# GATB/gatb-core

Hardware: AMD Instinct MI355X
Metric: distinct k-mers/s at k=31 (higher is better)
Workload: dtype u64

## Files before the change

gatb-core_amd/csrc/gkc_common.hpp:

```cpp
#pragma once
#include <hip/hip_runtime.h>
#include <stdint.h>
#include <stdio.h>
#include <stdlib.h>
#include <stdarg.h>
#include <string.h>
#include <string>
#include <vector>
#include <chrono>
#include <map>
#include <atomic>
#include <mutex>
#include <condition_variable>
#include <thread>
#include <algorithm>
#include "../../include/gkc.h"

struct gkc_error { int code; std::string msg; };

#define GKC_FAIL(ctx, code_, ...) do { (ctx)->set_error((code_), __VA_ARGS__); return (code_); } while (0)
#define GKC_HIP(ctx, call) do { hipError_t e_ = (call); if (e_ != hipSuccess) { \
    (ctx)->set_error(e_ == hipErrorOutOfMemory ? GKC_ERR_NOMEM : GKC_ERR_HIP, "%s failed: %s (%s:%d)", #call, hipGetErrorString(e_), __FILE__, __LINE__); \
    return e_ == hipErrorOutOfMemory ? GKC_ERR_NOMEM : GKC_ERR_HIP; } } while (0)
#define GKC_TRY(expr) do { int rc_ = (expr); if (rc_ != GKC_OK) return rc_; } while (0)

constexpr uint64_t GKC_PASS_GATHERED = 0x6761746865726564ull;
constexpr int SCAN_THREADS = 512;
constexpr int SCAN_PER_THREAD = 16;
constexpr int SCAN_TILE = SCAN_THREADS * SCAN_PER_THREAD;
constexpr int DESC_START_BITS = 13, DESC_NBK_BITS = 6;
static_assert(SCAN_TILE == (1 << DESC_START_BITS), "descriptor start field");
constexpr uint32_t DESC_PARTS_MAX = 1u << (32 - DESC_START_BITS - DESC_NBK_BITS);
constexpr uint32_t SCAN_COARSE_MAX = 4096;
constexpr int SCAN_HALO_WORDS = 4;
constexpr int SCAN_WORDS = SCAN_TILE / 16 + SCAN_HALO_WORDS;

constexpr int MAX_SUB_BITS = 13;
constexpr int MAX_SUB = 1 << MAX_SUB_BITS;
constexpr int SUB_TARGET = 512;

struct GkcTun {
    uint32_t scan_coarse_max; uint64_t push_split, push_chunk; bool scan_global_atomics, refine_recompute, scan_no_desc;
    int weight_bits, dedupe, max_sub_bits, lanes; uint64_t slice_min, batch_keys; bool slices, batch_lpt, no_f64; uint32_t wg_max, scatter_wgs, deep_bits, sink_first_div;
    bool sink_packed, sink_packed2, sink_width6, sink_two_widths, sink_debug; int sink_adaptive; uint64_t sink_dense; int unpack_threads;
    bool bloom_atomic, bloom_gather, mphf_regions, mphf_ordered; uint64_t bloom_query_regions_min, mphf_regions_min;
    uint64_t query_index_stride;
    int vmm; uint32_t vmm_chunk_mb, vmm_min_mb; bool vmm_with_rccl, pool_debug, pool_trace, verbose; double filebox_timeout; char fault[32];
    static const char* raw(const char* name) { return getenv(name); }
    static long long num(const char* name, long long dflt) { const char* e = raw(name); return e && *e ? atoll(e) : dflt; }
    static bool on(const char* name) { return raw(name) != nullptr; }
    static bool not0(const char* name) { const char* e = raw(name); return !(e && atoi(e) == 0); }
    void read() {
        scan_coarse_max = (uint32_t)std::max<long long>(1, num("GKC_SCAN_COARSE_MAX", SCAN_COARSE_MAX));
        push_split = (uint64_t)std::max<long long>(1024, num("GKC_PUSH_SPLIT", 16000000000ll)); push_chunk = (uint64_t)std::max<long long>(64, num("GKC_PUSH_CHUNK", 1ll << 30));
        scan_global_atomics = on("GKC_SCAN_GLOBAL_ATOMICS"); refine_recompute = on("GKC_REFINE_RECOMPUTE"); scan_no_desc = on("GKC_SCAN_NO_DESC");
        weight_bits = (int)num("GKC_WEIGHT_BITS", 0); dedupe = (int)num("GKC_DEDUPE", -1); max_sub_bits = (int)num("GKC_MAX_SUB_BITS", -1); lanes = (int)num("GKC_STAGEB_LANES", 2);
        slice_min = (uint64_t)std::max<long long>(1, num("GKC_SLICE_MIN", 8000000)); batch_keys = (uint64_t)num("GKC_BATCH_KEYS", 0);
        slices = not0("GKC_SLICES"); batch_lpt = not0("GKC_BATCH_LPT"); no_f64 = on("GKC_NO_F64");
        wg_max = (uint32_t)num("GKC_WG_MAX", 0); scatter_wgs = (uint32_t)std::max<long long>(1, num("GKC_SCATTER_WGS", 176)); deep_bits = (uint32_t)std::max<long long>(1, num("GKC_DEEP_BITS", MAX_SUB_BITS));
        sink_first_div = (uint32_t)std::max<long long>(1, num("GKC_SINK_FIRST_DIV", 4));
        sink_packed = not0("GKC_SINK_PACKED"); sink_packed2 = not0("GKC_SINK_PACKED2"); sink_width6 = not0("GKC_SINK_WIDTH6"); sink_debug = on("GKC_SINK_DEBUG"); sink_adaptive = (int)num("GKC_SINK_ADAPTIVE", 1);
        sink_two_widths = not0("GKC_SINK_TWO_WIDTHS");
        sink_dense = (uint64_t)num("GKC_SINK_DENSE", 0); unpack_threads = (int)num("GKC_UNPACK_THREADS", 0);
        bloom_atomic = on("GKC_BLOOM_ATOMIC"); bloom_gather = on("GKC_BLOOM_GATHER"); mphf_regions = not0("GKC_MPHF_REGIONS"); mphf_ordered = on("GKC_MPHF_ORDERED");
        bloom_query_regions_min = (uint64_t)num("GKC_BLOOM_QUERY_REGIONS_MIN", 2000000); mphf_regions_min = (uint64_t)num("GKC_MPHF_REGIONS_MIN", 1ll << 21);
        query_index_stride = (uint64_t)std::min<long long>(1ll << 40, std::max<long long>(1, num("GKC_QUERY_INDEX_STRIDE", 256)));
        vmm = (int)num("GKC_VMM", 1); vmm_chunk_mb = (uint32_t)std::max<long long>(2, num("GKC_VMM_CHUNK_MB", 1024)); vmm_min_mb = (uint32_t)std::max<long long>(1, num("GKC_VMM_MIN_MB", 64));
        vmm_with_rccl = num("GKC_VMM_WITH_RCCL", 0) == 1; pool_debug = on("GKC_POOL_DEBUG"); pool_trace = on("GKC_POOL_TRACE"); verbose = on("GKC_VERBOSE");
        filebox_timeout = raw("GKC_FILEBOX_TIMEOUT") ? atof(raw("GKC_FILEBOX_TIMEOUT")) : 600.0; memset(fault, 0, sizeof fault); if (raw("GKC_FAULT")) strncpy(fault, raw("GKC_FAULT"), sizeof fault - 1);
    }
};
inline GkcTun& gkc_tun() { static GkcTun t = [] { GkcTun x; x.read(); return x; }(); return t; }
inline void gkc_tun_refresh() { static std::mutex mu; std::lock_guard<std::mutex> lk(mu); GkcTun x; x.read(); gkc_tun() = x; }

inline thread_local hipStream_t tl_stream_ = nullptr;

struct VmmBlock { size_t bytes = 0; std::vector<hipMemGenericAllocationHandle_t> handles; std::vector<size_t> sizes; };
struct DevPool {
    std::recursive_mutex mu;
    std::multimap<size_t, void*> cache;
    std::map<void*, size_t> live;
    std::map<void*, VmmBlock> vmm;
    int device = 0; bool vmm_ok = true; size_t vmm_gran = 0; int vmm_state = 0;
    hipError_t raw_alloc(void** out, size_t want) {
        if (vmm_state == 0) {
            vmm_state = -1;
            int sup = 0;
            if (gkc_tun().vmm != 0 && hipDeviceGetAttribute(&sup, hipDeviceAttributeVirtualMemoryManagementSupported, device) == hipSuccess && sup) {
                hipMemAllocationProp prop{}; prop.type = hipMemAllocationTypePinned; prop.location.type = hipMemLocationTypeDevice; prop.location.id = device;
                if (hipMemGetAllocationGranularity(&vmm_gran, &prop, hipMemAllocationGranularityRecommended) == hipSuccess && vmm_gran) vmm_state = 1;
            }
            (void)hipGetLastError();
        }
        if (vmm_state != 1 || !vmm_ok || want < ((size_t)gkc_tun().vmm_min_mb << 20)) return hipMalloc(out, want);
        const size_t total = (want + vmm_gran - 1) / vmm_gran * vmm_gran;
        void* base = nullptr;
        hipError_t e = hipMemAddressReserve(&base, total, 0, nullptr, 0);
        if (e != hipSuccess) { (void)hipGetLastError(); return hipMalloc(out, want); }
        hipMemAllocationProp prop{}; prop.type = hipMemAllocationTypePinned; prop.location.type = hipMemLocationTypeDevice; prop.location.id = device;
        VmmBlock B; B.bytes = total;
        size_t off = 0;
        const size_t chunk_bytes = (size_t)gkc_tun().vmm_chunk_mb << 20;
        const bool dbg = gkc_tun().pool_debug;
        double t_create = 0, t_map = 0, t_access = 0;
        auto now = [] { return std::chrono::steady_clock::now(); };
        auto ms = [](std::chrono::steady_clock::time_point a, std::chrono::steady_clock::time_point b) { return std::chrono::duration<double, std::milli>(b - a).count(); };
        while (off < total && e == hipSuccess) {
            const size_t n = std::min(std::max(chunk_bytes / vmm_gran, (size_t)1) * vmm_gran, total - off);
            hipMemGenericAllocationHandle_t h;
            const auto t0 = now();
            e = hipMemCreate(&h, n, &prop, 0);
            const auto t1 = now();
            if (e == hipSuccess) { e = hipMemMap((char*)base + off, n, 0, h, 0); if (e != hipSuccess) (void)hipMemRelease(h); }
            t_create += ms(t0, t1); t_map += ms(t1, now());
            if (e == hipSuccess) { B.handles.push_back(h); B.sizes.push_back(n); off += n; }
// ... 265 lines not shown
```

gatb-core_amd/csrc/gkc_sink.hip:

```cpp
#include "gkc_common.hpp"
#include "gkc_device.hpp"
#include "gkc_wire.hpp"
#include <algorithm>
#include <utility>
#include <atomic>
#include <deque>
#include <pthread.h>
#include <sched.h>
#include <sys/syscall.h>
#include <unistd.h>

namespace { constexpr uint32_t PK_THREADS = 256; }

struct PackPlan { const uint32_t* blk_first;  const uint64_t* ptot;  uint32_t nb; };
struct PackOut {
    uint64_t* bases; uint32_t* cb_off; uint32_t* pay_off16; uint8_t* wbits;
    uint8_t* payload; unsigned long long* pay_cursor ;
    uint8_t* cb_stream; unsigned long long* cb_cursor;
    uint64_t* exc; unsigned long long* n_exc; uint32_t exc_cap;
};

struct PackBlock { uint64_t r0; uint32_t n; };
__device__ __forceinline__ PackBlock pack_block(const PackPlan& P, const uint32_t g)
{
    __shared__ uint32_t s_p;
    if (threadIdx.x == 0) {
        uint32_t lo = 0, hi = P.nb;
        while (hi - lo > 1) { const uint32_t mid = (lo + hi) >> 1; if (P.blk_first[mid] <= g) lo = mid; else hi = mid; }
        s_p = lo;
    }
    __syncthreads();
    const uint32_t p = s_p, j = g - P.blk_first[p];
    const uint64_t s1 = P.ptot[2 * (p + 1) + 1], r0 = P.ptot[2 * p + 1] + (uint64_t)j * PK_BLOCK;
    return { r0, (uint32_t)min((uint64_t)PK_BLOCK, s1 - r0) };
}
__device__ __forceinline__ void pack_except(const PackOut& O, const uint64_t tag, const uint64_t value)
{
    const unsigned long long e = atomicAdd(O.n_exc, 1ull);
    if (e < O.exc_cap) { O.exc[2 * e] = tag; O.exc[2 * e + 1] = value; }
}
__device__ __forceinline__ void pack_words16(uint8_t* dst, const void* lds, const uint32_t words)
{
    for (uint32_t w = threadIdx.x; w < words; w += PK_THREADS) reinterpret_cast<uint4*>(dst)[w] = reinterpret_cast<const uint4*>(lds)[w];
}
struct PkvLds {
    __attribute__((aligned(16))) unsigned long long bits[PK_BLOCK / 64];
    __attribute__((aligned(16))) uint8_t cb[PK_BLOCK];
    uint32_t wcnt[PK_THREADS / 64];
    unsigned long long base, pay;
};
__device__ __forceinline__ void pkv_clear(PkvLds& S) { for (uint32_t i = threadIdx.x; i < PK_BLOCK / 64; i += PK_THREADS) S.bits[i] = 0ull; }
__device__ __forceinline__ uint32_t pkv_abundance_round(const PackOut& O, PkvLds& S, const bool valid, const uint32_t ab, const uint64_t rec, const uint32_t i0, const uint32_t run)
{
    const uint32_t lane = threadIdx.x & 63, wave = threadIdx.x >> 6;
    uint32_t ab8 = valid ? ab : 1u;
    if (ab8 >= 255u) { pack_except(O, rec, ab); ab8 = 255u; }
    const bool flag = ab8 != 1u;
    const unsigned long long bal = __ballot(flag);
    if (lane == 0) { S.bits[(i0 >> 6) + wave] = bal; S.wcnt[wave] = (uint32_t)__popcll(bal); }
    __syncthreads();
    uint32_t before = run, total = 0;
#pragma unroll
    for (int w = 0; w < PK_THREADS / 64; w++) { if (w < (int)wave) before += S.wcnt[w]; total += S.wcnt[w]; }
    if (flag) S.cb[before + (uint32_t)__popcll(bal & ((1ull << lane) - 1ull))] = (uint8_t)ab8;
    return run + total;
}
__device__ __forceinline__ uint8_t* pkv_reserve(const PackOut& O, PkvLds& S, const uint32_t g, const uint32_t bytes, const uint32_t run)
// ... 149 lines not shown
#pragma unroll
        for (int d_ = 32; d_ >= 1; d_ >>= 1) { const uint32_t y = __shfl_xor(wd, d_, 64); wd = y > wd ? y : wd; }
        if (lane == 0 && wd) atomicMax(&s_w[(i0 >> 7) + (wave >> 1)], wd);
        run = pkv_abundance_round(O, S, i < n, ab, r0 + i, i0, run);
        __syncthreads();
    }
    if (t < PKV_NSUB) {
        uint32_t W = K::sent(s_w[t]);
        if (t * PKV_SUB >= n) W = 0u;
        uint32_t x = 16u * W;
#pragma unroll
        for (int d_ = 1; d_ < 64; d_ <<= 1) { const uint32_t y = __shfl_up(x, d_, 64); if ((int)lane >= d_) x += y; }
        s_w[t] = W; s_off[t] = x - 16u * W;
        if (t == PKV_NSUB - 1) s_off[PKV_NSUB] = x;
        O.wbits[(uint64_t)g * PKV_NSUB + t] = (uint8_t)W;
    }
    __syncthreads();
    uint8_t* dstp = pkv_reserve(O, S, g, s_off[PKV_NSUB] + (uint32_t)PKV_BITMAP, run);
    for (uint32_t c0 = 0; c0 < n; c0 += PKV_CHUNK) {
        for (uint32_t i = t; i < PKV_CHUNK; i += PK_THREADS) K::put(s_key, 1 + i, c0 + i < n ? K::key(recs, r0 + c0 + i) : (key_t)0);
        if (t == 0) K::put(s_key, 0, K::key(recs, c0 ? r0 + c0 - 1 : r0));
        __syncthreads();
        const uint32_t sub0 = c0 / PKV_SUB, sub = sub0 + (t >> 4), W = s_w[sub], cbase = s_off[sub0];
        {
            unsigned __int128 acc = 0; uint32_t nbits = 0;
            uint8_t* o = s_out + (s_off[sub] - cbase) + (size_t)(t & 15u) * W;
            key_t prev = K::get(s_key, 8 * t);
#pragma unroll
            for (int q = 0; q < 8; q++) {
                const uint32_t i = c0 + 8 * t + q;
                const key_t key = K::get(s_key, 1 + 8 * t + q);
                const key_t d = i < n ? key - prev : (key_t)0;
                prev = key;
                K::append(acc, nbits, o, d, W);
            }
        }
        __syncthreads();
        pack_words16(dstp + cbase, s_out, (s_off[sub0 + PKV_CHUNK / PKV_SUB] - cbase) >> 4);
        __syncthreads();
    }
    pack_words16(dstp + s_off[PKV_NSUB], S.bits, (uint32_t)PKV_BITMAP / 16);
    pkv_flush_abundances(O, S, run);
}

__global__ __launch_bounds__(PK_THREADS) void k_pack_pkv_two_widths(const uint64_t* __restrict__ recs, PackPlan P, PackOut O)
{
    constexpr uint32_t NCH = PK_BLOCK / PKV_CHUNK, SPC = PKV_CHUNK / PKV_SUB;
    constexpr uint32_t OUT_WORDS = (uint32_t)(PKVT_CHUNK_MAX / 8) + 2;
    __shared__ __attribute__((aligned(16))) unsigned long long s_out[OUT_WORDS];
    __shared__ uint64_t s_key[PKV_CHUNK + 1];
    __shared__ PkvLds S;
    __shared__ unsigned long long s_wmax[2];
    __shared__ uint32_t s_hist[2][64];
    __shared__ uint32_t s_wl[PKV_NSUB], s_ws[PKV_NSUB], s_ns[PKV_NSUB], s_sz[PKV_NSUB];
    __shared__ uint32_t s_off[PKV_NSUB], s_choff[NCH + 1];
    const uint32_t g = blockIdx.x, t = threadIdx.x, lane = t & 63, wave = t >> 6;
    pkv_clear(S);
    if (t < PKV_NSUB) { s_wl[t] = 0u; s_ws[t] = 0u; s_ns[t] = 0u; s_sz[t] = 0u; }
    if (t < 128) s_hist[t >> 6][t & 63] = 0u;
    if (t < 2) s_wmax[t] = 0ull;
    const PackBlock B = pack_block(P, g);
    const uint64_t r0 = B.r0; const uint32_t n = B.n;
    if (t == 0) O.bases[g] = recs[2 * r0];
    uint32_t run = 0;
    for (uint32_t i0 = 0; i0 < n; i0 += PK_THREADS) {
        const uint32_t i = i0 + t, sb = wave >> 1;
        uint32_t ab = 1; uint64_t d = 0;
        if (i < n) {
            const ulonglong2 me = *reinterpret_cast<const ulonglong2*>(recs + 2 * (r0 + i));
            const uint64_t prev = i ? recs[2 * (r0 + i - 1)] : me.x;
            d = me.x - prev;
            ab = (uint32_t)me.y;
            const uint32_t len = d ? 64u - (uint32_t)__clzll((long long)d) : 0u;
            atomicAdd(&s_hist[sb][len < 63u ? len : 63u], 1u);
        }
#pragma unroll
        for (int d_ = 32; d_ >= 1; d_ >>= 1) { const uint64_t y = (uint64_t)__shfl_xor((unsigned long long)d, d_, 64); d = y > d ? y : d; }
        if (lane == 0 && d) atomicMax(&s_wmax[sb], (unsigned long long)d);
        run = pkv_abundance_round(O, S, i < n, ab, r0 + i, i0, run);
        if ((wave & 1u) == 0u) {
            const uint32_t sub = (i0 >> 7) + sb, first = sub * PKV_SUB, cnt = first < n ? min(PKV_SUB, n - first) : 0u;
            const uint64_t m = s_wmax[sb];
            uint32_t wl = m ? 64u - (uint32_t)__clzll((long long)m) : 0u;
            if (wl > 56u) wl = 64u;
            uint32_t cum = s_hist[sb][lane];
#pragma unroll
            for (int d_ = 1; d_ < 64; d_ <<= 1) { const uint32_t y = __shfl_up(cum, d_, 64); if ((int)lane >= d_) cum += y; }
            const uint32_t one = (cnt * wl + 7u) >> 3;
            uint32_t best = lane < wl && lane <= 56u ? ((PKV_SEL + ((cum * lane + 7u) >> 3) + (((cnt - cum) * wl + 7u) >> 3)) << 6) | lane : ~0u;
#pragma unroll
            for (int d_ = 32; d_ >= 1; d_ >>= 1) { const uint32_t y = __shfl_xor(best, d_, 64); best = y < best ? y : best; }
            const bool split = best != ~0u && (best >> 6) + 16u <= one;
            const uint32_t ws = split ? best & 63u : wl, ns = __shfl(cum, (int)(best & 63u), 64);
            if (lane == 0) { s_wl[sub] = wl; s_ws[sub] = ws; s_ns[sub] = split ? ns : 0u; s_sz[sub] = split ? best >> 6 : one; s_wmax[sb] = 0ull; }
            s_hist[sb][lane] = 0u;
        }
        __syncthreads();
    }
    if (t < PKV_NSUB) {
        const uint32_t sz = s_sz[t];
        uint32_t x = sz;
#pragma unroll
        for (int d_ = 1; d_ < (int)SPC; d_ <<= 1) { const uint32_t y = __shfl_up(x, d_, SPC); if ((int)(lane & (SPC - 1)) >= d_) x += y; }
        const uint32_t ct = (__shfl(x, (int)(lane | (SPC - 1)), 64) + 15u) & ~15u;
        uint32_t base = 0, end = 0;
#pragma unroll
        for (uint32_t c = 0; c < NCH; c++) { const uint32_t v = __shfl(ct, (int)(c * SPC), 64); if (c < lane / SPC) base += v; end += v; }
        s_off[t] = base + x - sz;
        if ((lane & (SPC - 1)) == 0) s_choff[lane / SPC] = base;
        if (t == 0) s_choff[NCH] = end;
        O.wbits[(uint64_t)g * 2 * PKV_NSUB + t] = (uint8_t)s_wl[t];
        O.wbits[(uint64_t)g * 2 * PKV_NSUB + PKV_NSUB + t] = (uint8_t)s_ws[t];
    }
    __syncthreads();
    uint8_t* dstp = pkv_reserve(O, S, g, s_choff[NCH] + (uint32_t)PKV_BITMAP, run);
    pack_words16(dstp, S.bits, (uint32_t)PKV_BITMAP / 16);
    dstp += PKV_BITMAP;
    auto put = [&](const uint32_t bit, const uint64_t v, const uint32_t w) {
        if (!v) return;
        const uint32_t sh = bit & 63u;
        atomicOr(&s_out[bit >> 6], (unsigned long long)(v << sh));
        if (sh + w > 64u) atomicOr(&s_out[(bit >> 6) + 1], (unsigned long long)(v >> (64u - sh)));
    };
    for (uint32_t c0 = 0, ch = 0; c0 < n; c0 += PKV_CHUNK, ch++) {
        const uint32_t cbase = s_choff[ch], cbytes = s_choff[ch + 1] - cbase;
        for (uint32_t i = t; i < PKV_CHUNK; i += PK_THREADS) s_key[1 + i] = c0 + i < n ? recs[2 * (r0 + c0 + i)] : 0ull;
        if (t == 0) s_key[0] = c0 ? recs[2 * (r0 + c0 - 1)] : recs[2 * r0];
        for (uint32_t w = t; w < (cbytes >> 3) + 2u; w += PK_THREADS) s_out[w] = 0ull;
        __syncthreads();
        {
            const uint32_t sub = ch * SPC + (t >> 4), wl = s_wl[sub], ws = s_ws[sub], ns = s_ns[sub], sbyte = s_off[sub] - cbase;
            const bool split = ws != wl;
            uint64_t dl[8]; uint32_t valid = 0, sel = 0;
            uint64_t prev = s_key[8 * t];
#pragma unroll
            for (int q = 0; q < 8; q++) {
                const uint32_t i = c0 + 8 * t + q;
                const uint64_t key = s_key[1 + 8 * t + q];
                dl[q] = i < n ? key - prev : 0ull;
                prev = key;
                const uint32_t len = dl[q] ? 64u - (uint32_t)__clzll((long long)dl[q]) : 0u;
                if (i < n) { valid |= 1u << q; if (!split || len > ws) sel |= 1u << q; }
            }
            const uint32_t mine = (uint32_t)__popc(sel) | ((uint32_t)__popc(valid) << 16);
            uint32_t x = mine;
#pragma unroll
            for (int d_ = 1; d_ < 16; d_ <<= 1) { const uint32_t y = __shfl_up(x, d_, 16); if ((int)(t & 15u) >= d_) x += y; }
            x -= mine;
            const uint32_t pl = x & 0xFFFFu, ps = (x >> 16) - pl;
            uint32_t sbit = 8u * (sbyte + PKV_SEL) + ps * ws;
            uint32_t lbit = 8u * (sbyte + (split ? PKV_SEL + ((ns * ws + 7u) >> 3) : 0u)) + pl * wl;
            if (split) put(8u * (sbyte + (t & 15u)), (uint64_t)sel, 8u);
#pragma unroll
            for (int q = 0; q < 8; q++) {
                if (!((valid >> q) & 1u)) continue;
                if ((sel >> q) & 1u) { put(lbit, dl[q], wl); lbit += wl; } else { put(sbit, dl[q], ws); sbit += ws; }
            }
        }
        __syncthreads();
        pack_words16(dstp + cbase, s_out, cbytes >> 4);
        __syncthreads();
    }
    pkv_flush_abundances(O, S, run);
}

struct SinkBatch {
    int users = 0;
    hipEvent_t copied = nullptr;
    hipEvent_t copy_start = nullptr;
    WireBatch w;
    uint64_t n_cb = 0;
    void* d_packed = nullptr;
    bool ready = false, syncing = false;
    std::atomic<uint64_t> next{0}, finished{0};
    std::atomic<bool> done{false};
    std::chrono::steady_clock::time_point t_queued, t_ready;
    double pack_ms = 0;
};

struct gkc_unpacker {
    gkc_ctx* c = nullptr;
    std::vector<std::thread> threads;
    std::mutex mu; std::condition_variable cv, cv_done;
    std::deque<SinkBatch*> queue;
    std::vector<SinkBatch*> all;
    bool stop = false;
    bool debug = false;
    uint8_t* staging = nullptr; uint64_t staging_cap = 0, staging_used = 0;
    std::atomic<uint64_t> n_decisions{0}, n_adaptive_raw{0}, max_batch_records{0};

    void worker()
    {
        (void)hipSetDevice(c->device);
        for (;;) {
            SinkBatch* B = nullptr;
            {   std::unique_lock<std::mutex> lk(mu);
                for (;;) {
                    if (stop) return;
                    if (!queue.empty()) {
                        B = queue.front();
                        if (B->ready) break;
                        if (!B->syncing) { B->syncing = true; break; }
                    }
                    cv.wait(lk);
                }
                B->users++;
            }
            if (!B->ready) {
                (void)hipEventSynchronize(B->copied);
// ... 147 lines not shown
static thread_local const char* g_sink_why = "";
bool gkc_sink_host_behind(gkc_ctx* c, uint64_t n_records, const GkcTun& tun)
{
    gkc_unpacker* U = c->unpacker;
    if (!U || !tun.sink_adaptive) return false;
    uint64_t pending = 0;
    {   std::lock_guard<std::mutex> lk(U->mu);
        for (SinkBatch* B : U->all) {
            if (B->done.load()) continue;
            if (B->ready || hipEventQuery(B->copied) == hipSuccess) pending += B->w.nblk - std::min<uint64_t>(B->finished.load(), B->w.nblk);
        }
    }
    (void)hipGetLastError();
    uint64_t ref = U->max_batch_records.load(); if (n_records > ref) { U->max_batch_records = n_records; ref = n_records; }
    const bool behind = tun.sink_adaptive == 2 ? (U->n_decisions++ & 1) != 0
                                                     : pending * PK_BLOCK > std::max<uint64_t>(ref + ref / 2, (uint64_t)1 << 22);
    if (behind) { g_sink_why = "the host is behind with the expansion (landed, unexpanded records beyond 1.5 batches): this batch travels raw"; U->n_adaptive_raw++; }
    return behind;
}

const char* gkc_sink_last_refusal() { return g_sink_why; }
void* gkc_sink_send_packed(gkc_ctx* c, const void* d_out, const uint64_t* d_ptot, const std::vector<uint64_t>& solid_prefix, uint8_t* h_dest, const GkcTun& tun)
{
    gkc_unpacker* U = c->unpacker;
    g_sink_why = "no staging buffer";
    if (!U || !U->staging) return nullptr;
    const uint32_t nb = (uint32_t)solid_prefix.size() - 1;
    std::vector<uint32_t> blk_first(nb + 1);
    uint64_t nblk = 0;
    for (uint32_t i = 0; i < nb; i++) { blk_first[i] = (uint32_t)nblk; nblk += (solid_prefix[i + 1] - solid_prefix[i] + PK_BLOCK - 1) / PK_BLOCK; }
    blk_first[nb] = (uint32_t)nblk;
    g_sink_why = "no records / too many blocks";
    if (nblk == 0 || nblk >= (1ull << 31)) return nullptr;
    const uint64_t dense_min = tun.sink_dense ? tun.sink_dense : PK_DENSE;
    const bool wide = c->key_words == 2;
    const uint64_t n_rec = solid_prefix[nb];
    const bool dense = n_rec / std::max<uint32_t>(nb, 1) >= (wide ? std::min<uint64_t>(dense_min, PK2_DENSE) : dense_min);
    const bool pkv_ok = tun.sink_width6 && !c->sink_no6 && n_rec < (1ull << 32);
    const WireFormat fmt = wide ? (pkv_ok ? WireFormat::Pkv16 : dense ? WireFormat::Fixed16 : WireFormat::Fixed17)
                         : !dense ? WireFormat::Fixed8 : !(c->amin <= 1 && pkv_ok) ? WireFormat::Fixed7 : tun.sink_two_widths ? WireFormat::PkvTwoWidths : WireFormat::Pkv;
    const bool pkv = wire_pkv(fmt);
    const WireLayout L = wire_layout(fmt, nblk, n_rec);
    g_sink_why = "no device memory for the packed copy";
    DevBuf d_first; if (c->ensure(d_first, (size_t)(nb + 1) * 4) != GKC_OK) return nullptr;
    uint8_t* d_packed = (uint8_t*)c->dalloc((size_t)L.total);
    if (!d_packed) return nullptr;
    hipStream_t st = cur_stream(c);
    const auto t_pack0 = std::chrono::steady_clock::now();
    unsigned long long* d_cnt = reinterpret_cast<unsigned long long*>(d_packed + L.cnt_off);
    unsigned long long h_cnt[3] = {0, 0, 0};
    bool ok = hipMemcpyAsync(d_first.p, blk_first.data(), (size_t)(nb + 1) * 4, hipMemcpyHostToDevice, st) == hipSuccess
           && hipMemsetAsync(d_cnt, 0, 24, st) == hipSuccess;
    if (ok) {
        const PackPlan P{ (const uint32_t*)d_first.p, d_ptot, nb };
        const PackOut O{ (uint64_t*)d_packed, (uint32_t*)(d_packed + L.cboff_off), (uint32_t*)(d_packed + L.payoff_off), d_packed + L.wbits_off, d_packed + L.pay_off, d_cnt + 2,
                         d_packed + L.cb_off, d_cnt + 1, (uint64_t*)(d_packed + L.exc_off), d_cnt, (uint32_t)L.exc_cap };
        auto launch = [&](auto kernel) { hipLaunchKernelGGL(kernel, dim3((unsigned)nblk), dim3(PK_THREADS), 0, st, (const uint64_t*)d_out, P, O); };
        switch (fmt) {
        case WireFormat::Fixed7: launch(k_pack_fixed<7>); break;
        case WireFormat::Fixed8: launch(k_pack_fixed<8>); break;
        case WireFormat::Pkv: launch(k_pack_pkv<1>); break;
        case WireFormat::PkvTwoWidths: launch(k_pack_pkv_two_widths); break;
        case WireFormat::Fixed16: launch(k_pack_fixed16<16>); break;
        case WireFormat::Fixed17: launch(k_pack_fixed16<17>); break;
        case WireFormat::Pkv16: launch(k_pack_pkv<2>); break;
        }
        ok = hipGetLastError() == hipSuccess && hipMemcpyAsync(h_cnt, d_cnt, 24, hipMemcpyDeviceToHost, st) == hipSuccess && hipStreamSynchronize(st) == hipSuccess;
    }
    d_first.release();
    const unsigned long long h_nexc = h_cnt[0], h_ncb = h_cnt[1], h_pay = h_cnt[2];
    g_sink_why = !ok ? "pack launch failed" : "too many exceptions";
    if (!ok || h_nexc > L.exc_cap || h_ncb > L.cb_cap || (pkv && h_pay > L.pay_cap - WIRE_TAIL)) { (void)hipGetLastError(); c->dfree(d_packed); return nullptr; }
    if (pkv && (double)(h_pay + h_ncb) > (wide ? 16.0 : 7.0) * (double)n_rec) c->sink_no6 = true;
    const WireLayout S = wire_staged(fmt, L, h_pay, h_ncb, h_nexc);
    SinkBatch* B = new SinkBatch();
    {   std::lock_guard<std::mutex> lk(c->mu);
        if (U->staging_used + S.total > U->staging_cap) { g_sink_why = "staging buffer full"; delete B; c->dfree(d_packed); return nullptr; }
        B->w.stage = U->staging + U->staging_used; U->staging_used += wire_round(S.total);
        c->sink_wire_bytes += S.pay_off + S.pay_cap + h_ncb + h_nexc * 16;
    }
    B->w.lay = S; B->w.fmt = fmt; B->w.nblk = nblk; B->w.dest = h_dest; B->n_cb = h_ncb; B->d_packed = d_packed;
    B->w.blk_rec0.resize(nblk); B->w.blk_n.resize(nblk);
    for (uint32_t i = 0; i < nb; i++) {
        const uint64_t s0 = solid_prefix[i], s1 = solid_prefix[i + 1];
        for (uint64_t r = s0, g = blk_first[i]; r < s1; r += PK_BLOCK, g++) { B->w.blk_rec0[g] = r; B->w.blk_n[g] = (uint32_t)std::min<uint64_t>(PK_BLOCK, s1 - r); }
    }
    if (tun.sink_debug && hipEventCreate(&B->copy_start) == hipSuccess) (void)hipEventRecord(B->copy_start, c->copy_stream);
    bool queued = hipEventCreateWithFlags(&B->copied, tun.sink_debug ? hipEventDefault : hipEventDisableTiming) == hipSuccess
               && hipMemcpyAsync((void*)B->w.stage, d_packed, (size_t)(S.pay_off + S.pay_cap), hipMemcpyDeviceToHost, c->copy_stream) == hipSuccess
               && (h_ncb == 0 || hipMemcpyAsync((void*)(B->w.stage + S.cb_off), d_packed + L.cb_off, (size_t)h_ncb, hipMemcpyDeviceToHost, c->copy_stream) == hipSuccess)
               && (h_nexc == 0 || hipMemcpyAsync((void*)(B->w.stage + S.exc_off), d_packed + L.exc_off, (size_t)h_nexc * 16, hipMemcpyDeviceToHost, c->copy_stream) == hipSuccess)
               && hipEventRecord(B->copied, c->copy_stream) == hipSuccess;
    if (!queued) { g_sink_why = "copy could not be queued"; (void)hipGetLastError(); (void)hipStreamSynchronize(c->copy_stream); if (B->copied) (void)hipEventDestroy(B->copied); delete B; c->dfree(d_packed); return nullptr; }
    B->t_queued = std::chrono::steady_clock::now(); B->pack_ms = std::chrono::duration<double, std::milli>(B->t_queued - t_pack0).count();
    if (tun.sink_debug) { std::lock_guard<std::mutex> lk(U->mu); if (U->all.empty()) fprintf(stderr, "[gkc sink] first batch queued %.1f ms after Stage B began\n", std::chrono::duration<double, std::milli>(B->t_queued - c->t_stage_b0).count()); }
    { std::lock_guard<std::mutex> lk(U->mu); U->all.push_back(B); U->queue.push_back(B); }
    U->cv.notify_all();
    return B;
}
```

gatb-core_amd/csrc/gkc_wire.hpp:

```cpp
#pragma once
#include <algorithm>
#include <cstdint>
#include <cstring>
#include <utility>
#include <vector>
#include <immintrin.h>

#if defined(__clang__)
#define GKC_WIRE_UNROLL _Pragma("unroll")
#else
#define GKC_WIRE_UNROLL _Pragma("GCC unroll 8")
#endif

constexpr uint32_t PK_BLOCK = 8192;
constexpr uint64_t pk_slot(int W) { return (uint64_t)PK_BLOCK * (uint64_t)W; }
constexpr uint64_t pk_esc(int W) { return (1ull << (8 * (W - 1))) - 1ull; }
constexpr uint64_t PK_KEY_EXC = 1ull << 63;
constexpr uint64_t PK_DENSE = 300000;
constexpr uint64_t PK_KEY_EXC_HI = (1ull << 63) | (1ull << 62);
constexpr uint64_t PK2_DENSE = 100000;
constexpr uint32_t PKV_CHUNK = 2048, PKV_SUB = 128, PKV_NSUB = PK_BLOCK / PKV_SUB;
constexpr uint64_t PKV_BITMAP = PK_BLOCK / 8;
constexpr uint32_t PKV_SEL = PKV_SUB / 8;
constexpr uint64_t PKVT_CHUNK_MAX = (uint64_t)(PKV_CHUNK / PKV_SUB) * (PKV_SEL + PKV_SUB * 8);

enum class WireFormat : int { Fixed7, Fixed8, Pkv, PkvTwoWidths, Fixed16, Fixed17, Pkv16 };
constexpr bool wire_pkv(WireFormat f) { return f == WireFormat::Pkv || f == WireFormat::PkvTwoWidths || f == WireFormat::Pkv16; }
constexpr bool wire_key16(WireFormat f) { return f == WireFormat::Fixed16 || f == WireFormat::Fixed17 || f == WireFormat::Pkv16; }
constexpr int wire_entry(WireFormat f) { return f == WireFormat::Fixed7 ? 7 : f == WireFormat::Fixed8 ? 8 : f == WireFormat::Fixed16 ? 16 : f == WireFormat::Fixed17 ? 17 : 0; }
constexpr uint64_t wire_block_max(WireFormat f)
{
    return f == WireFormat::Pkv ? (uint64_t)PK_BLOCK * 8 + PKV_BITMAP : f == WireFormat::PkvTwoWidths ? (uint64_t)PK_BLOCK * 8 + (uint64_t)PKV_NSUB * PKV_SEL + PKV_BITMAP
         : f == WireFormat::Pkv16 ? (uint64_t)PK_BLOCK * 16 + PKV_BITMAP : pk_slot(wire_entry(f));
}

constexpr uint64_t WIRE_ALIGN = 64, WIRE_TAIL = 64;
constexpr uint32_t WIRE_EXC_CAP = 1u << 20;
constexpr uint64_t wire_round(uint64_t x) { return (x + WIRE_ALIGN - 1) / WIRE_ALIGN * WIRE_ALIGN; }
struct WireLayout {
    uint64_t cboff_off = 0, payoff_off = 0, wbits_off = 0;
    uint64_t pay_off = 0, pay_cap = 0;
    uint64_t cb_off = 0, cb_cap = 0;
    uint64_t exc_off = 0, exc_cap = 0;
    uint64_t cnt_off = 0;
    uint64_t total = 0;
    uint64_t block_max = 0;
};
constexpr WireLayout wire_layout(WireFormat f, uint64_t nblk, uint64_t n_rec)
{
    WireLayout L;
    const bool pkv = wire_pkv(f);
    L.block_max = wire_block_max(f);
    L.cboff_off = wire_round(nblk * (wire_key16(f) ? 16 : 8));
    L.payoff_off = L.cboff_off + (pkv ? wire_round(nblk * 4) : 0);
    L.wbits_off = L.payoff_off + (pkv ? wire_round(nblk * 4) : 0);
    L.pay_off = L.wbits_off + (pkv ? nblk * PKV_NSUB * (f == WireFormat::PkvTwoWidths ? 2 : 1) : 0);
    L.pay_cap = nblk * L.block_max + WIRE_TAIL;
    L.cb_off = L.pay_off + L.pay_cap; L.cb_cap = pkv ? wire_round(n_rec) : 0;
    L.exc_off = L.cb_off + L.cb_cap; L.exc_cap = WIRE_EXC_CAP;
    L.cnt_off = L.exc_off + L.exc_cap * 16;
    L.total = L.cnt_off + WIRE_TAIL;
    return L;
}
constexpr WireLayout wire_staged(WireFormat f, WireLayout L, uint64_t pay_cursor, uint64_t n_cb, uint64_t n_exc)
{
    if (wire_pkv(f)) L.pay_cap = wire_round(pay_cursor);
    L.cb_off = L.pay_off + L.pay_cap; L.cb_cap = wire_round(n_cb);
    L.exc_off = L.cb_off + L.cb_cap; L.exc_cap = n_exc;
    L.cnt_off = L.exc_off + n_exc * 16;
    L.total = L.cnt_off + WIRE_TAIL;
    return L;
}
constexpr uint64_t wire_staging_bytes(int key_words, uint64_t sink_bytes, uint64_t nb_partitions)
{
    return key_words == 1 ? sink_bytes / 16 * 8 + (sink_bytes / 16 / PKV_SUB + nb_partitions * PKV_NSUB) * 2 + nb_partitions * (wire_block_max(WireFormat::PkvTwoWidths) + 8) + ((uint64_t)64 << 20)
                          : sink_bytes / 32 * 17 + nb_partitions * (wire_block_max(WireFormat::Fixed17) + 16) + ((uint64_t)64 << 20);
}
// ... 98 lines not shown
        const uint32_t m = (uint32_t)(bits[i >> 6] >> (i & 63)) & 255u;
GKC_WIRE_UNROLL
        for (int j = 0; j < 8; j++) { uint64_t w; memcpy(&w, q + ((j * W) >> 3), 8); one(i + j, w, (uint32_t)((j * W) & 7), (m >> j) & 1u); }
    }
    for (uint64_t bit = (uint64_t)i * W; i < cnt; i++, bit += W) { uint64_t w; memcpy(&w, pay + (bit >> 3), 8); one(i, w, (uint32_t)(bit & 7), (uint32_t)(bits[i >> 6] >> (i & 63)) & 1u); }
}
typedef void (*pkv_fn)(const WireBatch&, const uint8_t*, uint32_t, uint64_t, uint64_t&, const uint64_t*, const uint8_t*&, __m128i*);
template <size_t... I> const pkv_fn* pkv_table(std::index_sequence<I...>) { static const pkv_fn t[] = { &pkv_sub<(int)I>... }; return t; }
inline void unpack_pkv(const WireBatch& B, uint64_t g)
{
    static const pkv_fn* const table = pkv_table(std::make_index_sequence<65>());
    PkvBlock K = pkv_block(B, g);
    uint64_t key = K.base[0];
    __m128i* out = reinterpret_cast<__m128i*>(B.dest + K.r0 * 16);
    for (uint32_t s0 = 0; s0 < K.n; s0 += PKV_SUB) {
        const uint32_t W = std::min<uint32_t>(K.wb[s0 / PKV_SUB], 64u);
        table[W](B, K.pay, std::min<uint32_t>(PKV_SUB, K.n - s0), K.r0 + s0, key, K.bits + (s0 >> 6), K.cb, out + s0);
        K.pay += 16u * W;
    }
}
inline void unpack_pkv16(const WireBatch& B, uint64_t g)
{
    typedef unsigned __int128 u128;
    PkvBlock K = pkv_block(B, g);
    u128 key = ((u128)K.base[1] << 64) | K.base[0];
    __m128i* out = reinterpret_cast<__m128i*>(B.dest + K.r0 * 32);
    for (uint32_t s0 = 0; s0 < K.n; s0 += PKV_SUB) {
        const uint32_t W = K.wb[s0 / PKV_SUB], wl = W < 64u ? W : 64u, wh = W - wl;
        const uint64_t ml = wl >= 64 ? ~0ull : (1ull << wl) - 1ull, mh = wh >= 64 ? ~0ull : (1ull << wh) - 1ull;
        uint64_t bit = 0;
        const uint32_t e = std::min<uint32_t>(K.n, s0 + PKV_SUB);
        for (uint32_t i = s0; i < e; i++) {
            u128 x; memcpy(&x, K.pay + (bit >> 3), 16);
            const uint64_t lo = (uint64_t)(x >> (bit & 7)) & ml; bit += wl;
            uint64_t hi = 0;
            if (wh) { memcpy(&x, K.pay + (bit >> 3), 16); hi = (uint64_t)(x >> (bit & 7)) & mh; bit += wh; }
            key += ((u128)hi << 64) | lo;
            wire_store(out + 2 * (size_t)i, key, wire_abundance(B, (uint32_t)(K.bits[i >> 6] >> (i & 63)) & 1u, K.cb, K.r0 + i));
        }
        K.pay += 16u * W;
    }
}
template <int W> void pkv_take(const uint8_t* p, const uint32_t cnt, uint64_t* d)
{
    constexpr uint64_t mask = W >= 64 ? ~0ull : ((1ull << (W & 63)) - 1ull);
    uint32_t i = 0;
    for (; i + 8 <= cnt; i += 8) {
        const uint8_t* q = p + (size_t)(i >> 3) * W;
GKC_WIRE_UNROLL
        for (int j = 0; j < 8; j++) { uint64_t w; memcpy(&w, q + ((j * W) >> 3), 8); d[i + j] = (w >> ((j * W) & 7)) & mask; }
    }
    for (uint64_t bit = (uint64_t)i * W; i < cnt; i++, bit += W) { uint64_t w; memcpy(&w, p + (bit >> 3), 8); d[i] = (w >> (bit & 7)) & mask; }
}
typedef void (*take_fn)(const uint8_t*, uint32_t, uint64_t*);
template <size_t... I> const take_fn* take_table(std::index_sequence<I...>) { static const take_fn t[] = { &pkv_take<(int)I>... }; return t; }
inline void pkv_merge(const WireBatch& B, const uint64_t* sd, const uint64_t* ld, uint32_t si, uint32_t li, const uint64_t* sel, uint32_t i, const uint32_t cnt, const uint64_t rec0,
                      uint64_t& key, const uint64_t* bits, const uint8_t*& cb, __m128i* out)
{
    for (; i < cnt; i++) {
        const uint32_t l = (uint32_t)(sel[i >> 6] >> (i & 63)) & 1u, f = (uint32_t)(bits[i >> 6] >> (i & 63)) & 1u;
        key += l ? ld[li] : sd[si]; li += l; si += 1u - l;
        wire_store(out + i, key, wire_abundance(B, f, cb, rec0 + i));
    }
}
inline bool have_avx512() { static const bool ok = __builtin_cpu_supports("avx512f") && __builtin_cpu_supports("popcnt"); return ok; }
#if !defined(__HIP_DEVICE_COMPILE__)
__attribute__((target("avx512f,popcnt")))
inline void pkv_emit512(const WireBatch& B, const uint64_t* sd, const uint64_t* ld, const uint64_t* sel, const uint32_t cnt, const uint64_t rec0, uint64_t& key_io,
                        const uint64_t* bits, const uint8_t*& cb_io, __m128i* out)
{
    const __m512i zero = _mm512_setzero_si512(), one = _mm512_set1_epi64(1), esc255 = _mm512_set1_epi64(255), last = _mm512_set1_epi64(7);
    const __m512i i0 = _mm512_setr_epi64(0, 8, 1, 9, 2, 10, 3, 11), i1 = _mm512_setr_epi64(4, 12, 5, 13, 6, 14, 7, 15);
    const bool aligned = ((uintptr_t)out & 63) == 0;
    __m512i carry = _mm512_set1_epi64((long long)key_io);
    const uint8_t* cb = cb_io;
    uint32_t si = 0, li = 0, i = 0;
    for (; i + 8 <= cnt; i += 8) {
        const __mmask8 m = (__mmask8)(sel[i >> 6] >> (i & 63)), fm = (__mmask8)(bits[i >> 6] >> (i & 63));
        __m512i x = _mm512_mask_expand_epi64(_mm512_maskz_expand_epi64((__mmask8)~m, _mm512_loadu_si512(sd + si)), m, _mm512_loadu_si512(ld + li));
        const uint32_t nl = (uint32_t)__builtin_popcount(m); li += nl; si += 8u - nl;
        x = _mm512_add_epi64(x, _mm512_alignr_epi64(x, zero, 7));
        x = _mm512_add_epi64(x, _mm512_alignr_epi64(x, zero, 6));
        x = _mm512_add_epi64(x, _mm512_alignr_epi64(x, zero, 4));
        x = _mm512_add_epi64(x, carry);
        carry = _mm512_permutexvar_epi64(last, x);
        __m512i ab = _mm512_mask_expand_epi64(one, fm, _mm512_cvtepu8_epi64(_mm_loadl_epi64(reinterpret_cast<const __m128i*>(cb))));
        cb += __builtin_popcount(fm);
        const __mmask8 esc = _mm512_cmpeq_epi64_mask(ab, esc255);
        if (esc) {
            alignas(64) uint64_t a8[8]; _mm512_store_si512(a8, ab);
            for (int j = 0; j < 8; j++) if ((esc >> j) & 1) a8[j] = (uint32_t)wire_lookup(B, rec0 + i + j);
            ab = _mm512_load_si512(a8);
        }
        const __m512i lo = _mm512_permutex2var_epi64(x, i0, ab), hi = _mm512_permutex2var_epi64(x, i1, ab);
        if (aligned) { _mm512_stream_si512(reinterpret_cast<__m512i*>(out + i), lo); _mm512_stream_si512(reinterpret_cast<__m512i*>(out + i + 4), hi); }
        else {
            _mm_stream_si128(out + i, _mm512_castsi512_si128(lo)); _mm_stream_si128(out + i + 1, _mm512_extracti32x4_epi32(lo, 1));
            _mm_stream_si128(out + i + 2, _mm512_extracti32x4_epi32(lo, 2)); _mm_stream_si128(out + i + 3, _mm512_extracti32x4_epi32(lo, 3));
            _mm_stream_si128(out + i + 4, _mm512_castsi512_si128(hi)); _mm_stream_si128(out + i + 5, _mm512_extracti32x4_epi32(hi, 1));
            _mm_stream_si128(out + i + 6, _mm512_extracti32x4_epi32(hi, 2)); _mm_stream_si128(out + i + 7, _mm512_extracti32x4_epi32(hi, 3));
        }
    }
    key_io = (uint64_t)_mm_cvtsi128_si64(_mm512_castsi512_si128(carry)); cb_io = cb;
    pkv_merge(B, sd, ld, si, li, sel, i, cnt, rec0, key_io, bits, cb_io, out);
}
#else
void pkv_emit512(const WireBatch&, const uint64_t*, const uint64_t*, const uint64_t*, uint32_t, uint64_t, uint64_t&, const uint64_t*, const uint8_t*&, __m128i*);
#endif
inline void unpack_pkv_two_widths(const WireBatch& B, uint64_t g, const bool avx512)
{
    static const take_fn* const take = take_table(std::make_index_sequence<65>());
    const PkvBlock K = pkv_block(B, g);
    const uint8_t* cb = K.cb;
    uint64_t key = K.base[0];
    __m128i* out = reinterpret_cast<__m128i*>(B.dest + K.r0 * 16);
    uint32_t off = 0;
    for (uint32_t s0 = 0; s0 < K.n; s0 += PKV_SUB) {
        const uint32_t s = s0 / PKV_SUB, cnt = std::min<uint32_t>(PKV_SUB, K.n - s0);
        const uint32_t wl = std::min<uint32_t>(K.wb[s], 64u), ws = std::min<uint32_t>(K.wb[PKV_NSUB + s], 64u);
        uint64_t sel[2] = { ~0ull, ~0ull }; uint32_t ns = 0, sbytes = 0, skip = 0;
        if (ws != wl) {
            memcpy(sel, K.pay + off, PKV_SEL);
            const uint32_t nl = (uint32_t)(__builtin_popcountll(sel[0]) + __builtin_popcountll(sel[1]));
            ns = cnt - std::min(nl, cnt); sbytes = (ns * ws + 7u) >> 3; skip = PKV_SEL;
        }
        uint64_t d[2][PKV_SUB + 8];
        if (ns) take[ws](K.pay + off + skip, ns, d[0]);
        take[wl](K.pay + off + skip + sbytes, cnt - ns, d[1]);
        if (avx512) pkv_emit512(B, d[0], d[1], sel, cnt, K.r0 + s0, key, K.bits + (s0 >> 6), cb, out + s0);
        else pkv_merge(B, d[0], d[1], 0, 0, sel, 0, cnt, K.r0 + s0, key, K.bits + (s0 >> 6), cb, out + s0);
        off += skip + sbytes + (((cnt - ns) * wl + 7u) >> 3);
        if ((s & (PKV_CHUNK / PKV_SUB - 1)) == PKV_CHUNK / PKV_SUB - 1) off = (off + 15u) & ~15u;
    }
}
inline void unpack_block(const WireBatch& B, uint64_t g, const bool avx512)
{
    switch (B.fmt) {
    case WireFormat::Fixed7: unpack_fixed<7>(B, g); break;
    case WireFormat::Fixed8: unpack_fixed<8>(B, g); break;
    case WireFormat::Pkv: unpack_pkv(B, g); break;
    case WireFormat::PkvTwoWidths: unpack_pkv_two_widths(B, g, avx512); break;
    case WireFormat::Fixed16: unpack_fixed16<16>(B, g); break;
    case WireFormat::Fixed17: unpack_fixed16<17>(B, g); break;
    case WireFormat::Pkv16: unpack_pkv16(B, g); break;
    }
}
```

Baseline: 8.209 billion.

## Add power-of-four gap coding for sorted k-mer deltas in two-width packer

Adds a third sub-block encoding to the two-width packed sink. Gaps of the form c·4^e (c<4) are stored as one byte each, and other gaps are stored at the long width. The packer counts such gaps per sub-block and picks this coding when it gives fewer bytes than the split coding, and the host unpacker decodes it with an AVX-512 or scalar path. The aim is a smaller wire payload to transfer, at the cost of an extra ballot and atomic per sub-block in the pack kernel plus a new decode branch. It is enabled by default through GKC_SINK_POWER_GAPS.

```diff
diff --git a/gatb-core_amd/csrc/gkc_common.hpp b/gatb-core_amd/csrc/gkc_common.hpp
--- a/gatb-core_amd/csrc/gkc_common.hpp
+++ b/gatb-core_amd/csrc/gkc_common.hpp
@@ -42,7 +42,7 @@
 struct GkcTun {
     uint32_t scan_coarse_max; uint64_t push_split, push_chunk; bool scan_global_atomics, refine_recompute, scan_no_desc;
     int weight_bits, dedupe, max_sub_bits, lanes; uint64_t slice_min, batch_keys; bool slices, batch_lpt, no_f64; uint32_t wg_max, scatter_wgs, deep_bits, sink_first_div;
-    bool sink_packed, sink_packed2, sink_width6, sink_two_widths, sink_debug; int sink_adaptive; uint64_t sink_dense; int unpack_threads;
+    bool sink_packed, sink_packed2, sink_width6, sink_two_widths, sink_power_gaps, sink_debug; int sink_adaptive; uint64_t sink_dense; int unpack_threads;
     bool bloom_atomic, bloom_gather, mphf_regions, mphf_ordered; uint64_t bloom_query_regions_min, mphf_regions_min;
     uint64_t query_index_stride;
     int vmm; uint32_t vmm_chunk_mb, vmm_min_mb; bool vmm_with_rccl, pool_debug, pool_trace, verbose; double filebox_timeout; char fault[32];
@@ -61,6 +61,7 @@
         sink_first_div = (uint32_t)std::max<long long>(1, num("GKC_SINK_FIRST_DIV", 4));
         sink_packed = not0("GKC_SINK_PACKED"); sink_packed2 = not0("GKC_SINK_PACKED2"); sink_width6 = not0("GKC_SINK_WIDTH6"); sink_debug = on("GKC_SINK_DEBUG"); sink_adaptive = (int)num("GKC_SINK_ADAPTIVE", 1);
         sink_two_widths = not0("GKC_SINK_TWO_WIDTHS");
+        sink_power_gaps = not0("GKC_SINK_POWER_GAPS");
         sink_dense = (uint64_t)num("GKC_SINK_DENSE", 0); unpack_threads = (int)num("GKC_UNPACK_THREADS", 0);
         bloom_atomic = on("GKC_BLOOM_ATOMIC"); bloom_gather = on("GKC_BLOOM_GATHER"); mphf_regions = not0("GKC_MPHF_REGIONS"); mphf_ordered = on("GKC_MPHF_ORDERED");
         bloom_query_regions_min = (uint64_t)num("GKC_BLOOM_QUERY_REGIONS_MIN", 2000000); mphf_regions_min = (uint64_t)num("GKC_MPHF_REGIONS_MIN", 1ll << 21);
diff --git a/gatb-core_amd/csrc/gkc_sink.hip b/gatb-core_amd/csrc/gkc_sink.hip
--- a/gatb-core_amd/csrc/gkc_sink.hip
+++ b/gatb-core_amd/csrc/gkc_sink.hip
@@ -12,7 +12,8 @@
 
 namespace { constexpr uint32_t PK_THREADS = 256; }
 
-struct PackPlan { const uint32_t* blk_first;  const uint64_t* ptot;  uint32_t nb; };
+struct PackPlan { const uint32_t* blk_first;  const uint64_t* ptot;  uint32_t nb;
+                  uint32_t power_gaps;  };
 struct PackOut {
     uint64_t* bases; uint32_t* cb_off; uint32_t* pay_off16; uint8_t* wbits;
     uint8_t* payload; unsigned long long* pay_cursor ;
@@ -268,13 +269,14 @@
     __shared__ PkvLds S;
     __shared__ unsigned long long s_wmax[2];
     __shared__ uint32_t s_hist[2][64];
+    __shared__ uint32_t s_npow[2];
     __shared__ uint32_t s_wl[PKV_NSUB], s_ws[PKV_NSUB], s_ns[PKV_NSUB], s_sz[PKV_NSUB];
     __shared__ uint32_t s_off[PKV_NSUB], s_choff[NCH + 1];
     const uint32_t g = blockIdx.x, t = threadIdx.x, lane = t & 63, wave = t >> 6;
     pkv_clear(S);
     if (t < PKV_NSUB) { s_wl[t] = 0u; s_ws[t] = 0u; s_ns[t] = 0u; s_sz[t] = 0u; }
     if (t < 128) s_hist[t >> 6][t & 63] = 0u;
-    if (t < 2) s_wmax[t] = 0ull;
+    if (t < 2) { s_wmax[t] = 0ull; s_npow[t] = 0u; }
     const PackBlock B = pack_block(P, g);
     const uint64_t r0 = B.r0; const uint32_t n = B.n;
     if (t == 0) O.bases[g] = recs[2 * r0];
@@ -290,6 +292,10 @@
             const uint32_t len = d ? 64u - (uint32_t)__clzll((long long)d) : 0u;
             atomicAdd(&s_hist[sb][len < 63u ? len : 63u], 1u);
         }
+        if (P.power_gaps) {
+            const unsigned long long pw = __ballot(i < n && wire_power_code(d) != 255u);
+            if (lane == 0 && pw) atomicAdd(&s_npow[sb], (uint32_t)__popcll(pw));
+        }
 #pragma unroll
         for (int d_ = 32; d_ >= 1; d_ >>= 1) { const uint64_t y = (uint64_t)__shfl_xor((unsigned long long)d, d_, 64); d = y > d ? y : d; }
         if (lane == 0 && d) atomicMax(&s_wmax[sb], (unsigned long long)d);
@@ -307,8 +313,11 @@
 #pragma unroll
             for (int d_ = 32; d_ >= 1; d_ >>= 1) { const uint32_t y = __shfl_xor(best, d_, 64); best = y < best ? y : best; }
             const bool split = best != ~0u && (best >> 6) + 16u <= one;
-            const uint32_t ws = split ? best & 63u : wl, ns = __shfl(cum, (int)(best & 63u), 64);
-            if (lane == 0) { s_wl[sub] = wl; s_ws[sub] = ws; s_ns[sub] = split ? ns : 0u; s_sz[sub] = split ? best >> 6 : one; s_wmax[sb] = 0ull; }
+            const uint32_t two = split ? best >> 6 : one;
+            const uint32_t npow = min(s_npow[sb], cnt), pbytes = PKV_SEL + npow + (((cnt - npow) * wl + 7u) >> 3);
+            const bool power = P.power_gaps && pbytes + 16u <= one && pbytes < two;
+            const uint32_t ws = power ? PKV_WS_POWER : split ? best & 63u : wl, ns = __shfl(cum, (int)(best & 63u), 64);
+            if (lane == 0) { s_wl[sub] = wl; s_ws[sub] = ws; s_ns[sub] = power ? npow : split ? ns : 0u; s_sz[sub] = power ? pbytes : two; s_wmax[sb] = 0ull; s_npow[sb] = 0u; }
             s_hist[sb][lane] = 0u;
         }
         __syncthreads();
@@ -346,7 +355,8 @@
         __syncthreads();
         {
             const uint32_t sub = ch * SPC + (t >> 4), wl = s_wl[sub], ws = s_ws[sub], ns = s_ns[sub], sbyte = s_off[sub] - cbase;
-            const bool split = ws != wl;
+            const bool split = ws != wl, power = ws == PKV_WS_POWER;
+            const uint32_t wsb = power ? 8u : ws;
             uint64_t dl[8]; uint32_t valid = 0, sel = 0;
             uint64_t prev = s_key[8 * t];
 #pragma unroll
@@ -355,8 +365,9 @@
                 const uint64_t key = s_key[1 + 8 * t + q];
                 dl[q] = i < n ? key - prev : 0ull;
                 prev = key;
-                const uint32_t len = dl[q] ? 64u - (uint32_t)__clzll((long long)dl[q]) : 0u;
-                if (i < n) { valid |= 1u << q; if (!split || len > ws) sel |= 1u << q; }
+                const uint32_t len = dl[q] ? 64u - (uint32_t)__clzll((long long)dl[q]) : 0u, code = wire_power_code(dl[q]);
+                if (i < n) { valid |= 1u << q; if (!split || (power ? code == 255u : len > ws)) sel |= 1u << q; }
+                if (power && code != 255u) dl[q] = code;
             }
             const uint32_t mine = (uint32_t)__popc(sel) | ((uint32_t)__popc(valid) << 16);
             uint32_t x = mine;
@@ -364,13 +375,13 @@
             for (int d_ = 1; d_ < 16; d_ <<= 1) { const uint32_t y = __shfl_up(x, d_, 16); if ((int)(t & 15u) >= d_) x += y; }
             x -= mine;
             const uint32_t pl = x & 0xFFFFu, ps = (x >> 16) - pl;
-            uint32_t sbit = 8u * (sbyte + PKV_SEL) + ps * ws;
-            uint32_t lbit = 8u * (sbyte + (split ? PKV_SEL + ((ns * ws + 7u) >> 3) : 0u)) + pl * wl;
+            uint32_t sbit = 8u * (sbyte + PKV_SEL) + ps * wsb;
+            uint32_t lbit = 8u * (sbyte + (split ? PKV_SEL + ((ns * wsb + 7u) >> 3) : 0u)) + pl * wl;
             if (split) put(8u * (sbyte + (t & 15u)), (uint64_t)sel, 8u);
 #pragma unroll
             for (int q = 0; q < 8; q++) {
                 if (!((valid >> q) & 1u)) continue;
-                if ((sel >> q) & 1u) { put(lbit, dl[q], wl); lbit += wl; } else { put(sbit, dl[q], ws); sbit += ws; }
+                if ((sel >> q) & 1u) { put(lbit, dl[q], wl); lbit += wl; } else { put(sbit, dl[q], wsb); sbit += wsb; }
             }
         }
         __syncthreads();
@@ -624,7 +635,7 @@
     bool ok = hipMemcpyAsync(d_first.p, blk_first.data(), (size_t)(nb + 1) * 4, hipMemcpyHostToDevice, st) == hipSuccess
            && hipMemsetAsync(d_cnt, 0, 24, st) == hipSuccess;
     if (ok) {
-        const PackPlan P{ (const uint32_t*)d_first.p, d_ptot, nb };
+        const PackPlan P{ (const uint32_t*)d_first.p, d_ptot, nb, tun.sink_power_gaps ? 1u : 0u };
         const PackOut O{ (uint64_t*)d_packed, (uint32_t*)(d_packed + L.cboff_off), (uint32_t*)(d_packed + L.payoff_off), d_packed + L.wbits_off, d_packed + L.pay_off, d_cnt + 2,
                          d_packed + L.cb_off, d_cnt + 1, (uint64_t*)(d_packed + L.exc_off), d_cnt, (uint32_t)L.exc_cap };
         auto launch = [&](auto kernel) { hipLaunchKernelGGL(kernel, dim3((unsigned)nblk), dim3(PK_THREADS), 0, st, (const uint64_t*)d_out, P, O); };
diff --git a/gatb-core_amd/csrc/gkc_wire.hpp b/gatb-core_amd/csrc/gkc_wire.hpp
--- a/gatb-core_amd/csrc/gkc_wire.hpp
+++ b/gatb-core_amd/csrc/gkc_wire.hpp
@@ -23,6 +23,19 @@
 constexpr uint64_t PKV_BITMAP = PK_BLOCK / 8;
 constexpr uint32_t PKV_SEL = PKV_SUB / 8;
 constexpr uint64_t PKVT_CHUNK_MAX = (uint64_t)(PKV_CHUNK / PKV_SUB) * (PKV_SEL + PKV_SUB * 8);
+constexpr uint32_t PKV_WS_POWER = 255;
+constexpr uint32_t wire_power_code(const uint64_t d)
+{
+    if (!d) return 0u;
+    const uint32_t e = (uint32_t)__builtin_ctzll(d) >> 1;
+    const uint64_t c = d >> (2u * e);
+    return c < 4u ? ((uint32_t)c << 5) | e : 255u;
+}
+constexpr uint64_t wire_power_delta(const uint32_t b) { return (uint64_t)((b >> 5) & 3u) << (2u * (b & 31u)); }
+static_assert(PKV_WS_POWER > 64 && PKV_WS_POWER < 256, "the power marker is a width byte no real width takes");
+static_assert(wire_power_code(0) == 0 && wire_power_code(1) == 32 && wire_power_code(3ull << 62) == 127 && wire_power_code(5) == 255 && wire_power_code(1ull << 63) == 95
+              && wire_power_delta(127) == 3ull << 62 && wire_power_delta(wire_power_code(2ull << 34)) == 2ull << 34, "power codes");
+static_assert(PKVT_CHUNK_MAX >= (uint64_t)(PKV_CHUNK / PKV_SUB) * (PKV_SEL + PKV_SUB * 8), "a power sub-block (16 + n_pow + at most 8 (cnt - n_pow) bytes) fits the chunk bound of a split one");
 
 enum class WireFormat : int { Fixed7, Fixed8, Pkv, PkvTwoWidths, Fixed16, Fixed17, Pkv16 };
 constexpr bool wire_pkv(WireFormat f) { return f == WireFormat::Pkv || f == WireFormat::PkvTwoWidths || f == WireFormat::Pkv16; }
@@ -227,6 +240,29 @@
     }
     for (uint64_t bit = (uint64_t)i * W; i < cnt; i++, bit += W) { uint64_t w; memcpy(&w, p + (bit >> 3), 8); d[i] = (w >> (bit & 7)) & mask; }
 }
+inline void pkv_take_power_scalar(const uint8_t* p, const uint32_t cnt, uint64_t* d)
+{
+    for (uint32_t i = 0; i < cnt; i += 8) {
+        uint64_t w; memcpy(&w, p + i, 8);
+GKC_WIRE_UNROLL
+        for (int j = 0; j < 8; j++) d[i + j] = wire_power_delta((uint32_t)(w >> (8 * j)) & 255u);
+    }
+}
+#if !defined(__HIP_DEVICE_COMPILE__)
+__attribute__((target("avx512f,popcnt")))
+inline void pkv_take_power512(const uint8_t* p, const uint32_t cnt, uint64_t* d)
+{
+    const __m512i m3 = _mm512_set1_epi64(3), m31 = _mm512_set1_epi64(31);
+    for (uint32_t i = 0; i < cnt; i += 8) {
+        const __m512i b = _mm512_cvtepu8_epi64(_mm_loadl_epi64(reinterpret_cast<const __m128i*>(p + i)));
+        const __m512i c = _mm512_and_si512(_mm512_srli_epi64(b, 5), m3), e2 = _mm512_slli_epi64(_mm512_and_si512(b, m31), 1);
+        _mm512_storeu_si512(d + i, _mm512_sllv_epi64(c, e2));
+    }
+}
+#else
+void pkv_take_power512(const uint8_t*, uint32_t, uint64_t*);
+#endif
+inline void pkv_take_power(const uint8_t* p, const uint32_t cnt, uint64_t* d, const bool avx512) { if (avx512) pkv_take_power512(p, cnt, d); else pkv_take_power_scalar(p, cnt, d); }
 typedef void (*take_fn)(const uint8_t*, uint32_t, uint64_t*);
 template <size_t... I> const take_fn* take_table(std::index_sequence<I...>) { static const take_fn t[] = { &pkv_take<(int)I>... }; return t; }
 inline void pkv_merge(const WireBatch& B, const uint64_t* sd, const uint64_t* ld, uint32_t si, uint32_t li, const uint64_t* sel, uint32_t i, const uint32_t cnt, const uint64_t rec0,
@@ -292,15 +328,16 @@
     uint32_t off = 0;
     for (uint32_t s0 = 0; s0 < K.n; s0 += PKV_SUB) {
         const uint32_t s = s0 / PKV_SUB, cnt = std::min<uint32_t>(PKV_SUB, K.n - s0);
-        const uint32_t wl = std::min<uint32_t>(K.wb[s], 64u), ws = std::min<uint32_t>(K.wb[PKV_NSUB + s], 64u);
+        const bool power = K.wb[PKV_NSUB + s] == PKV_WS_POWER;
+        const uint32_t wl = std::min<uint32_t>(K.wb[s], 64u), ws = power ? 8u : std::min<uint32_t>(K.wb[PKV_NSUB + s], 64u);
         uint64_t sel[2] = { ~0ull, ~0ull }; uint32_t ns = 0, sbytes = 0, skip = 0;
-        if (ws != wl) {
+        if (power || ws != wl) {
             memcpy(sel, K.pay + off, PKV_SEL);
             const uint32_t nl = (uint32_t)(__builtin_popcountll(sel[0]) + __builtin_popcountll(sel[1]));
             ns = cnt - std::min(nl, cnt); sbytes = (ns * ws + 7u) >> 3; skip = PKV_SEL;
         }
         uint64_t d[2][PKV_SUB + 8];
-        if (ns) take[ws](K.pay + off + skip, ns, d[0]);
+        if (ns) { if (power) pkv_take_power(K.pay + off + skip, ns, d[0], avx512); else take[ws](K.pay + off + skip, ns, d[0]); }
         take[wl](K.pay + off + skip + sbytes, cnt - ns, d[1]);
         if (avx512) pkv_emit512(B, d[0], d[1], sel, cnt, K.r0 + s0, key, K.bits + (s0 >> 6), cb, out + s0);
         else pkv_merge(B, d[0], d[1], 0, 0, sel, 0, cnt, K.r0 + s0, key, K.bits + (s0 >> 6), cb, out + s0);
```

Result: faster. 8.459 billion, median of 6 (+3.0%).
